# Picurit/cutter-vad

Hardware: AMD Instinct MI355X
Metric: 512-sample frames/sec, Silero V5 16kHz, batch=8192 streams per GPU (higher is better)
Workload: dtype f32

## Files before the change

### cutter_vad_amd/csrc/engine.cpp

```cpp
#include "../../include/vad_engine.h"

#include <hip/hip_runtime_api.h>

#include <algorithm>
#include <atomic>
#include <cmath>
#include <condition_variable>
#include <cstdarg>
#include <cstdlib>
#include <new>
#include <chrono>
#include <cstring>
#include <deque>
#include <mutex>
#include <string>
#include <thread>
#include <unordered_map>
#include <array>
#include <vector>

#include "pack_weights.h"
#include "resample_generic.h"
#include "vad_layout.h"

extern "C" hipError_t vadk_launch_silero_v5(const vadk::StepParams *p, hipStream_t stream);
extern "C" hipError_t vadk_launch_silero_v4(const vadk::StepParams *p, hipStream_t stream);
extern "C" hipError_t vadk_launch_silero_v5_t16(const vadk::StepParams *p, hipStream_t stream);
extern "C" hipError_t vadk_launch_silero_v4_t16(const vadk::StepParams *p, int one_per_cu, hipStream_t stream);
extern "C" hipError_t vadk_launch_silero_v5_t16_rates(const vadk::StepParams *p, const vadk::RateParams *r, hipStream_t stream);
extern "C" hipError_t vadk_launch_silero_v5_scan16(const vadk::StepParams *p, const vadk::ScanItem *items, const vadk::ScanArgs *a,
                                                   hipStream_t stream);
extern "C" hipError_t vadk_launch_scan_cut(const vadk::CutArgs *a, hipStream_t stream);
extern "C" hipError_t vadk_launch_scan_segments(const vadk::SegArgs *a, hipStream_t stream);
extern "C" hipError_t vadk_launch_scan_resample(const vadk::ScanResampleArgs *a, hipStream_t stream);
extern "C" hipError_t vadk_launch_resample(const vadk::ResampleParams *p, hipStream_t stream);
extern "C" hipError_t vadk_launch_slot_control(vadk::SmSlot *sm, float *state, const int32_t *d_slots, int n, int op,
                                               const vadk::SmSlot *def, const vad_thresholds *d_thr, int nthr, hipStream_t stream);
extern "C" hipError_t vadk_launch_sm_replay(vadk::SmSlot *sm, int slot, const float *probs, int n, uint8_t *events,
                                            int32_t *seg, hipStream_t stream);
extern "C" hipError_t vadk_launch_g711_expand(const void *d_in, int16_t *d_out, int64_t nbytes, int alaw, hipStream_t stream);

namespace {
// ... 98 lines not shown
    int16_t *d_g711 = nullptr; size_t d_g711_cap = 0;
    static constexpr size_t SMALL_BYTES = 256u << 10;
    uint8_t *h_small_in = nullptr, *h_small_out = nullptr;
    std::vector<void *> host_blocks;
    uint8_t *d_small_in = nullptr, *d_small_out = nullptr;
    vadk::StepParams base{};
    static constexpr int T16_MAX_STREAMS = 4096;
    float *d_wstream16 = nullptr;
    size_t wbytes16 = 0;
    float *d_wstream16x = nullptr;
    size_t wbytes16x = 0;
    float *d_wstream16y = nullptr;
    size_t wbytes16y = 0;
    uint32_t sect16[vadk::NWAVES][16] = {};
    int tile_policy = 0;
    bool rates_fused = true;
    bool shared_gpu = false;
    int sample_rate = 16000;
    int frame_samples = VAD_FRAME_SAMPLES;
    std::vector<int32_t> work_index;
    std::vector<uint8_t> work_kind;
    std::vector<int64_t> work_samples;
    uint8_t *h_ctl = nullptr, *d_ctl = nullptr; size_t ctl_cap = 0;
    static constexpr int PIPE_DEPTH = 2;
    struct PipeBuf {
        void *d_frames = nullptr; size_t d_frames_cap = 0;
        uint8_t *d_io = nullptr, *h_io = nullptr; size_t io_cap = 0;
        hipEvent_t copied = nullptr, done = nullptr, out = nullptr;
        int64_t ticket = -1; int64_t n = 0; int32_t T = 0; bool busy = false, collecting = false;
    } pipe[PIPE_DEPTH];
// ... 373 lines not shown
        p16.wstream_x_bytes = (uint32_t)e->wbytes16x;
        p16.wstream_y = e->d_wstream16y;
        p16.wstream_y_bytes = (uint32_t)e->wbytes16y;
        std::memcpy(p16.sect, e->sect16, sizeof p16.sect);
        const int tiles16 = (p.n + 15) / 16;
        r = vadk_launch_silero_v4_t16(&p16, (!e->shared_gpu && tiles16 <= e->prop.multiProcessorCount) ? 1 : 0, s);
    } else if (e->version == 5 && t16) {
        vadk::StepParams p16 = p;
        p16.wstream = e->d_wstream16;
        p16.wstream_bytes = (uint32_t)e->wbytes16;
        p16.wstream_x = e->d_wstream16x;
        p16.wstream_x_bytes = (uint32_t)e->wbytes16x;
        p16.wstream_y = e->d_wstream16y;
        p16.wstream_y_bytes = (uint32_t)e->wbytes16y;
        std::memcpy(p16.sect, e->sect16, sizeof p16.sect);
        r = vadk_launch_silero_v5_t16(&p16, s);
    } else if (e->version == 5) r = vadk_launch_silero_v5(&p, s);
    else if (e->version == 4) r = vadk_launch_silero_v4(&p, s);
    if (r != hipSuccess) return e->hip_fail(r, "kernel launch");
    e->steps += 1;
    e->frames += (int64_t)p.n * p.T;
    return VAD_OK;
}

int step_host(vad_engine *e, const int64_t *slots, int64_t n, int32_t T, const void *frames, int fmt, float thr,
              float *probs, uint8_t *events, int32_t *seg) {
    if (!e) return VAD_ERR_INVALID_ARG;
    std::lock_guard<std::mutex> lk(e->mu);
    if (n < 0 || T < 1 || (n > 0 && (!slots || !frames || !probs)))
        return e->fail(VAD_ERR_INVALID_ARG, "Model prediction failed: null buffer or bad count");
// ... 2611 lines not shown
            g_create_error = "vad_debug_pack_weights: output buffer too small";
            return VAD_ERR_INVALID_ARG;
        }
        std::memcpy(out, pw.data.data(), pw.data.size() * sizeof(float));
    }
    return VAD_OK;
}

int vad_debug_set_tile(vad_engine *e, int32_t streams_per_tile) {
    if (!e) return VAD_ERR_INVALID_ARG;
    std::lock_guard<std::mutex> lk(e->mu);
    if (streams_per_tile == -1 || streams_per_tile == -2) {
        e->rates_fused = streams_per_tile == -2;
        return VAD_OK;
    }
    if (streams_per_tile != 0 && streams_per_tile != 16 && streams_per_tile != 32)
        return e->fail(VAD_ERR_INVALID_ARG, "tile: 0 (by batch size), 16 or 32");
    if (streams_per_tile == 16 && !e->d_wstream16)
        return e->fail(VAD_ERR_UNSUPPORTED, "Silero V5's 8 kHz sub-model has no 16-stream tile kernel");
    e->tile_policy = streams_per_tile;
    return VAD_OK;
}

int vad_debug_sm_replay(vad_engine *e, int64_t slot, const float *probs, int64_t n, uint8_t *events_out,
                        int32_t *seg_frames_out) {
    if (!e || !probs || !events_out || !seg_frames_out || n < 1) return VAD_ERR_INVALID_ARG;
    std::lock_guard<std::mutex> lk(e->mu);
    if (slot < 0 || slot >= e->max_streams || !e->open[(size_t)slot])
        return e->fail(VAD_ERR_BAD_SLOT, "slot %lld is not an open stream", (long long)slot);
    HIP_TRY(e, hipSetDevice(e->device));
    if (int rc = ensure(e, e->d_probs, e->d_probs_cap, sizeof(float) * n)) return rc;
    if (int rc = ensure(e, e->d_events, e->d_events_cap, (size_t)n)) return rc;
    if (int rc = ensure(e, e->d_seg, e->d_seg_cap, sizeof(int32_t) * n)) return rc;
    HIP_TRY(e, hipMemcpyAsync(e->d_probs, probs, sizeof(float) * n, hipMemcpyHostToDevice, e->stream));
    HIP_TRY(e, hipStreamSynchronize(e->stream));
// ... 40 lines not shown
```

### cutter_vad_amd/csrc/silero_v5_t16.hip

```cpp
#include <hip/hip_runtime.h>
#include <type_traits>
#include <utility>
#include "vad_layout.h"
#include "sm_device.h"
#include "vadk_device.h"

using namespace vadk;

#ifdef VADK_STAMPS
#define STAMP(k)                                                                                   \
    do {                                                                                           \
        if (lane == 0) P.stamps[((size_t)blockIdx.x * NWAVES + w) * 32 + (k)] = clock64();          \
    } while (0)
template <class V>
__device__ __forceinline__ void stamp_wait(V v) {
    if constexpr (sizeof(V) == 4) asm volatile("" ::"v"(v) : "memory");
    else if constexpr (sizeof(V) == 32) asm volatile("" ::"v"(v.b.x) : "memory");
    else asm volatile("" ::"v"(v.x) : "memory");
}
#define STAMP_ON(k, v)                                                                             \
    do {                                                                                           \
        if constexpr (!RS) {                                                                       \
            stamp_wait(v);                                                                         \
            STAMP(k);                                                                              \
        }                                                                                          \
    } while (0)
#define STAMP_DRAIN(k)                                                                             \
// ... 82 lines not shown
        if constexpr (k_ == 7) { F_[0] = N_[0]; F_[1] = N_[1]; F_[2] = N_[2]; }                                 \
        if constexpr (!(FOLD(u)) || k_ == 7) SB();                                                              \
    }
#define X3_STEP(s, B, SRC, EXTRA, FOLD)                                                                         \
    X3_UNIT(8 * (s) + 0, B, SRC, EXTRA, FOLD) X3_UNIT(8 * (s) + 1, B, SRC, EXTRA, FOLD)                         \
    X3_UNIT(8 * (s) + 2, B, SRC, EXTRA, FOLD) X3_UNIT(8 * (s) + 3, B, SRC, EXTRA, FOLD)                         \
    X3_UNIT(8 * (s) + 4, B, SRC, EXTRA, FOLD) X3_UNIT(8 * (s) + 5, B, SRC, EXTRA, FOLD)                         \
    X3_UNIT(8 * (s) + 6, B, SRC, EXTRA, FOLD) X3_UNIT(8 * (s) + 7, B, SRC, EXTRA, FOLD)
#define X3_HALF(B, SRC, EXTRA, FOLD)                                                                            \
    {                                                                                                           \
        u32x4 F_[3], N_[3];                                                                                     \
        _Pragma("unroll") for (int p_ = 0; p_ < 3; ++p_) F_[p_] = PL_RD(SRC, 0, p_);                            \
        SB();                                                                                                   \
        X3_STEP(0, B, SRC, EXTRA, FOLD) X3_STEP(1, B, SRC, EXTRA, FOLD)                                         \
        X3_STEP(2, B, SRC, EXTRA, FOLD) X3_STEP(3, B, SRC, EXTRA, FOLD)                                         \
    }
#define X3_CONV(NS, NT, STR, NO, LDM, B, U0, SRC, ACC, EXTRA)                                         \
    {                                                                                                           \
        constexpr int NU_ = (NS) * 3 * (NT);                                                                    \
        u32x4 F_[3][3], N_[3][3];                                                                               \
        _Pragma("unroll") for (int c_ = 0; c_ < 3; ++c_)                                                        \
            _Pragma("unroll") for (int p_ = 0; p_ < 3; ++p_) F_[c_][p_] = PL_RD(SRC(c_), 0, p_);                \
        SB();                                                                                                   \
        x3_units([&](auto uc_) {                                                                                \
            constexpr int u_ = decltype(uc_)::value, s_ = u_ / (3 * (NT)), r_ = u_ % (3 * (NT));                \
            constexpr int t_ = r_ / (NT), tl_ = r_ % (NT);                                                      \
            if constexpr (u_ + X3_D < NU_) { LDM((B) + 3 * (u_ + X3_D), (U0) + u_ + X3_D) }                     \
            if constexpr (r_ == 0 && s_ + 1 < (NS)) {                                                           \
                _Pragma("unroll") for (int c_ = 0; c_ < 3; ++c_)                                                \
                    _Pragma("unroll") for (int p_ = 0; p_ < 3; ++p_) N_[c_][p_] = PL_RD(SRC(c_), s_ + 1, p_);   \
// ... 8 lines not shown
                    _Pragma("unroll") for (int c_ = 0; c_ < 3; ++c_)                                            \
                        _Pragma("unroll") for (int p_ = 0; p_ < 3; ++p_) F_[c_][p_] = N_[c_][p_];               \
                }                                                                                               \
            }                                                                                                   \
            SB();                                                                                               \
        }, std::make_integer_sequence<int, NU_>{});                                                             \
    }

#define STEP16_PARAMS const float *k_wstream, float *k_state, SmSlot *k_sm, const int32_t *k_slots, const void *k_frames, const int k_n, \
                      const uint32_t k_wstream_bytes, const int k_T, const StepParams P, const RateParams R
#define STEP16_NO_SCAN                                  \
    constexpr bool SCAN = false;                        \
    constexpr int CH = 1;                               \
    constexpr const ScanItem *k_items = nullptr;        \
    constexpr ScanArgs S{};
template <bool F32IN_, bool RS, bool K8 = false, bool ONE = false>
__global__ void __launch_bounds__(NTHREADS, 1) silero_v5_step16(STEP16_PARAMS) {
    constexpr int FMT = F32IN_ ? 0 : 1;
    STEP16_NO_SCAN
#include "silero_v5_t16_body.h"
}
template <bool ALAW, bool K8, bool ONE>
__global__ void __launch_bounds__(NTHREADS, 1) silero_v5_step16_g711(STEP16_PARAMS) {
    constexpr int FMT = ALAW ? 3 : 2;
    constexpr bool RS = false;
    STEP16_NO_SCAN
#include "silero_v5_t16_body.h"
}
template <int FMT_, bool K8>
__global__ void __launch_bounds__(NTHREADS, 1) silero_v5_scan16(const float *k_wstream, float *k_state, SmSlot *k_sm, const ScanItem *k_items,
                                                                const void *k_frames, const int k_n, const uint32_t k_wstream_bytes,
                                                                const int k_T, const StepParams P, const ScanArgs S) {
    constexpr int FMT = FMT_;
    constexpr bool RS = false, ONE = false, SCAN = true;
    constexpr int CH = 1;
    constexpr const int32_t *k_slots = nullptr;
    const RateParams R{};
#include "silero_v5_t16_body.h"
}
template <int FMT_, bool K8>
__global__ void __launch_bounds__(NTHREADS, 1) silero_v5_stereo16(const float *k_wstream, float *k_state, SmSlot *k_sm, const ScanItem *k_items,
                                                                  const void *k_frames, const int k_n, const uint32_t k_wstream_bytes,
                                                                  const int k_T, const StepParams P, const ScanArgs S) {
    constexpr int FMT = FMT_;
    constexpr bool RS = false, ONE = false, SCAN = true;
    constexpr int CH = 2;
    constexpr const int32_t *k_slots = nullptr;
    const RateParams R{};
#include "silero_v5_t16_body.h"
}
#undef STEP16_NO_SCAN
#undef STEP16_PARAMS
#undef X3_CONV
#undef X3_HALF
#undef X3_STEP
#undef X3_UNIT
#undef PL_RD


#define V5_ARGS p->wstream, p->state, p->sm, p->slots, p->frames, (int)p->n, p->wstream_bytes, (int)p->T, *p
extern "C" hipError_t vadk_launch_silero_v5_t16(const vadk::StepParams *p, hipStream_t stream) {
    (void)hipGetLastError();
    const int tiles = (p->n + MT16 - 1) / MT16;
    if (tiles <= 0) return hipSuccess;
    const vadk::RateParams none{};
#define T16_LAUNCH(F, K, O) hipLaunchKernelGGL((silero_v5_step16<F, false, K, O>), dim3(tiles), dim3(vadk::NTHREADS), 0, stream, V5_ARGS, none)
    if (p->T < 1) return hipErrorInvalidValue;
    const bool k8 = p->variant != 0;
// ... 10 lines not shown
            else { if (one) T16_LAUNCH_G711(false, false, true); else T16_LAUNCH_G711(false, false, false); }
        }
        return hipGetLastError();
    }
    if (p->fmt < 0 || p->fmt > 2) return hipErrorInvalidValue;
    const bool f32 = p->fmt == 0;
    if (k8) {
        if (f32) { if (one) T16_LAUNCH(true, true, true); else T16_LAUNCH(true, true, false); }
        else { if (one) T16_LAUNCH(false, true, true); else T16_LAUNCH(false, true, false); }
    } else {
        if (f32) { if (one) T16_LAUNCH(true, false, true); else T16_LAUNCH(true, false, false); }
        else { if (one) T16_LAUNCH(false, false, true); else T16_LAUNCH(false, false, false); }
    }
#undef T16_LAUNCH_G711
#undef T16_LAUNCH
    return hipGetLastError();
}

extern "C" hipError_t vadk_launch_silero_v5_scan16(const vadk::StepParams *p, const vadk::ScanItem *items, const vadk::ScanArgs *a,
                                                   hipStream_t stream) {
    (void)hipGetLastError();
    const int tiles = (p->n + MT16 - 1) / MT16;
    if (tiles <= 0) return hipSuccess;
    if (p->T < 1 || p->fmt < 0 || p->fmt > 4 || a->hopq < 1 || a->t0 < 0 || (a->audio_bytes >> 31)) return hipErrorInvalidValue;
    if ((reinterpret_cast<uintptr_t>(p->frames) & 3) || (reinterpret_cast<uintptr_t>(items) & 15)) return hipErrorInvalidValue;
    if (a->channels < 0 || a->channels > 2 || (a->channels == 2 && (reinterpret_cast<uintptr_t>(p->frames) & 7))) return hipErrorInvalidValue;
#define SCAN16_LAUNCH(F, K)                                                                                                    \
    hipLaunchKernelGGL((silero_v5_scan16<F, K>), dim3(tiles), dim3(vadk::NTHREADS), 0, stream, p->wstream, p->state, p->sm, items, \
                       p->frames, (int)p->n, p->wstream_bytes, (int)p->T, *p, *a)
#define STEREO16_LAUNCH(F, K)                                                                                                  \
// ... 27 lines not shown
```

### cutter_vad_amd/csrc/silero_v5_t16_body.h

```cpp
#define KP(f) k_##f
    using namespace vadk::v5;
    constexpr bool F32IN = FMT == 0;
    constexpr bool G711 = FMT >= 2;
    static_assert(!RS || F32IN, "resampled frames are float32");
    static_assert(!(RS && K8), "the fused resampler feeds the 16 kHz model");
    static_assert(!SCAN || (!RS && !ONE), "a scan is the frame-loop form on audio in HBM");
    static_assert(CH == 1 || (CH == 2 && SCAN), "two interleaved channels: whole recordings only");
    constexpr int QL = K8 ? 8 : 16;
    constexpr int CS = 4 * QL;
    constexpr int PP = K8 ? 24 : 48;
    __shared__ f32x4 lds[T_LDS_F4 + (RS ? MT16 * FQ : 0) + (F32IN ? T_FLAG_F4 : 0)];
    f32x4 *const RX = lds;
    f32x4 *const RE = lds + T_ROW_E * QSD;
    f32x4 *const RP0 = lds + T_ROW_E0 * QSD;
    f32x4 *const RH = lds + T_ROW_H * QSD;
    float *const headp = reinterpret_cast<float *>(RH + T_ROWS_H * QSD);
    float *const nyqv = headp + 64;
    float *const fcor = nyqv + 48;
    constexpr int FCOR_SINK = 144;
    SmSlot *const smL = reinterpret_cast<SmSlot *>(fcor + 144 + 64);
    f32x4 *const biasL = reinterpret_cast<f32x4 *>(smL + MT16);
    uint8_t *const flagL = reinterpret_cast<uint8_t *>(lds + T_LDS_F4 + (RS ? MT16 * FQ : 0));

    const int tid = threadIdx.x;
    const int lane = tid & 63;
    const int w = __builtin_amdgcn_readfirstlane(tid >> 6);
    if constexpr (!RS) STAMP(19);
    const int n = lane & 15;
    const int kq = lane >> 4;
    const int nq = kq * QSD + n;
    const int nqL = kq * QSL + n;
    const int vcol = (int)blockIdx.x * MT16 + n;
    int gf = vcol;
    bool live = vcol < KP(n);
    if constexpr (RS) {
        int s0 = R.seg[0].stream0, vs = 0;
#pragma unroll
        for (int k = 1; k < RATE_MAX_SEGS; ++k)
            if (k < R.nseg && vcol >= R.seg[k].vstart) { s0 = R.seg[k].stream0; vs = R.seg[k].vstart; }
        gf = s0 + vcol - vs;
        live = vcol < R.total;
    }
    const int tile0 = (int)blockIdx.x * MT16;
    int slot, ncol = 0;
    uint32_t obase = 0;
    if constexpr (SCAN) {
        const u32x4 it = live ? *reinterpret_cast<const u32x4 *>(k_items + vcol) : u32x4{0u, 0u, 0u, 0u};
        slot = (int)it.x;
        ncol = (int)it.z - S.t0;
        obase = it.w + (uint32_t)S.t0;
    } else {
        slot = live ? (KP(slots) ? KP(slots)[gf] : gf) : 0;
    }
    const __amdgpu_buffer_rsrc_t wrs = __builtin_amdgcn_make_buffer_rsrc(const_cast<float *>(KP(wstream)), 0, (int)KP(wstream_bytes), 0x00020000);
    const int lane16 = lane * 16;
#define WL(blk) ldw(wrs, lane16, (blk))
    const __amdgpu_buffer_rsrc_t wrx = __builtin_amdgcn_make_buffer_rsrc(const_cast<float *>(P.wstream_x), 0, (int)P.wstream_x_bytes, 0x00020000);
#define WX(blk) ldw(wrx, lane16, (blk))
// ... 21 lines not shown
        SCAN ? (int)S.audio_bytes : (int)((unsigned)KP(n) * (unsigned)T * ((f32in ? 2048u : G711 ? 512u : 1024u) >> (K8 ? 1 : 0))), 0x00020000);
    constexpr int X_NT = K8 ? 0 : 2;
    struct XQ2F { u32x4 a, b; };
    using XQ = std::conditional_t<CH == 2, std::conditional_t<f32in, XQ2F, std::conditional_t<G711, u32x2, u32x4>>,
                                  std::conditional_t<G711, uint32_t, u32x4>>;
    auto x_load = [&](int off) -> XQ {
        if constexpr (CH == 2 && f32in)
            return XQ2F{__builtin_amdgcn_raw_buffer_load_b128(frs, off, 0, X_NT), __builtin_amdgcn_raw_buffer_load_b128(frs, off + 16, 0, X_NT)};
        else if constexpr (CH == 2 && G711) return __builtin_amdgcn_raw_buffer_load_b64(frs, off, 0, X_NT);
        else if constexpr (G711) return __builtin_amdgcn_raw_buffer_load_b32(frs, off, 0, X_NT);
        else return __builtin_amdgcn_raw_buffer_load_b128(frs, off, 0, X_NT);
    };
    XQ xa_[4], xb_[4], xc_[4];
    constexpr bool XCARRY = !RS && !K8;
#define X_K0(c) ((XCARRY && (c) > 0) ? 2 : 0)
    f32x4 *const F4 = lds + T_LDS_F4;
    uint32_t xq0 = 0;
    [[maybe_unused]] uint32_t xmode = 0;
    if constexpr (SCAN) {
        const int li = tile0 + lms;
        if constexpr (CH == 2) {
            const uint32_t qm = li < KP(n) ? k_items[li].quad0 : 0u;
            xmode = qm >> SCAN_MODE_SHIFT;
            xq0 = (qm & ((1u << SCAN_MODE_SHIFT) - 1u)) + (uint32_t)S.t0 * S.hopq;
        } else {
        xq0 = (li < KP(n) ? k_items[li].quad0 : 0u) + (uint32_t)S.t0 * S.hopq;
        }
    }
#define X_ISSUE(c, XR, tt)                                                                                      \
    if constexpr (RS) {                                                                                         \
        _Pragma("unroll") for (int k = 0; k < 4; ++k)                                                           \
// ... 83 lines not shown
#pragma unroll
    for (int rt = 0; rt < 2; ++rt) hv[rt] = *reinterpret_cast<const f32x4 *>(KP(state) + (size_t)slot * 256 + 32 * w + 16 * rt + 4 * kq);
    SB();
    auto bias2 = __builtin_amdgcn_raw_buffer_load_b64(wrs, lane * 8, (o_l + T_LSTM_BIAS_BLOCK) * 1024, 0);
    const bool sm_thread = (tid < MT16) && live;
    const int sm_slot = slot;
    f32x4 smq[6];
    if (tid < MT16) {
#pragma unroll
        for (int k = 0; k < 6; ++k) smq[k] = reinterpret_cast<const f32x4 *>(KP(sm) + slot)[k];
    }
    SB();
    f32x4 xw[X3_NR][3];
#define X3_LDR(blk, slot) _Pragma("unroll") for (int p_ = 0; p_ < 3; ++p_) xw[(slot) % X3_NR][p_] = WL((blk) + p_);
#define X3_LD(B, u) X3_LDR((B) + 3 * (u), (u))
#define X3_LDX(blk, slot) _Pragma("unroll") for (int p_ = 0; p_ < 3; ++p_) xw[(slot) % X3_NR][p_] = WX((blk) + p_);
#define X3_LDY(blk, slot) _Pragma("unroll") for (int p_ = 0; p_ < 3; ++p_) xw[(slot) % X3_NR][p_] = WY((blk) + p_);
#define H_FIRSTX(tt)                                                                                            \
    {                                                                                                           \
        if constexpr (K8) { X_ISSUE8(0, xa_, tt) X_ISSUE8(2, xb_, tt) }                                         \
        else { X_ISSUE(0, xa_, tt) X_ISSUE(1, xb_, tt) }                                                        \
    }
#define H_FIRST(L, tt, WITHX)                                                                                   \
    {                                                                                                           \
        _Pragma("unroll") for (int u_ = 0; u_ < X3_D; ++u_) { X3_LD((L) + LSTM_X3_HALF_BLOCKS, u_) }             \
        if constexpr (WITHX) H_FIRSTX(tt)                                                                       \
        SB();                                                                                                   \
        if constexpr (RS) { X_ISSUE(2, xc_, tt) SB(); }                                                         \
    }
    if constexpr (!RS) STAMP(29);
    if constexpr (!RS) H_FIRST(o_x3, 0, K8)
    const f32x4 W1 = ldw(wrs, q * 16, o_nyq), W3 = ldw(wrs, (2 * QL + q) * 16, o_nyq);
    const float w64 = ldw(wrs, QL * 16, o_nyq).x;
    f32x4 cst[2];
#pragma unroll
    for (int rt = 0; rt < 2; ++rt) cst[rt] = *reinterpret_cast<const f32x4 *>(KP(state) + (size_t)slot * 256 + 128 + 32 * w + 16 * rt + 4 * kq);
    bool chunk0_requested = false;
    if constexpr (RS) {
        if (cur.valid && cur.S.wstream != nullptr && cur.S.n_in == 1536) {
            if (cur.shape == 0) load_chunk(std::integral_constant<int, 0>{}, cur, 0, xlA);
// ... 297 lines not shown
          else if (cur.shape == 1) run_part(std::integral_constant<int, 1>{});
          else if (cur.shape == 2) run_part(std::integral_constant<int, 2>{});
          else run_part(std::integral_constant<int, 3>{});
#undef OL
        }
        __syncthreads();
        cur = mk_part(cur.sk + 1);
        }
    }

    STAMP(0);
    for (int t = 0;;) {
        int ws_stft = o_stft, ws_x0 = o_x0, ws_y1 = o_y1, ws_e2 = o_e2, ws_e3 = o_e3, ws_l = o_l, ws_x3 = o_x3;
        asm volatile("" : "+s"(ws_stft), "+s"(ws_x0), "+s"(ws_y1), "+s"(ws_e2), "+s"(ws_e3), "+s"(ws_l), "+s"(ws_x3));
        f32x4 G[8];
        {
            const int wh = ws_x3 + LSTM_X3_HALF_BLOCKS;
            f32x4 xcA, xcB;
            float xm = 0.f;
            auto decode = [&](XQ b) -> f32x4 {
                f32x4 v;
                if constexpr (CH == 2) {
                    f32x4 dl, dr;
                    if constexpr (G711) {
                        dl = g711_quad<FMT == 3>(__builtin_amdgcn_perm(b.y, b.x, 0x06040200u));
                        dr = g711_quad<FMT == 3>(__builtin_amdgcn_perm(b.y, b.x, 0x07050301u));
                    } else if constexpr (!f32in) {
                        dl = f32x4{i16_div((int)(short)(b.x & 0xffffu), sc, rsc), i16_div((int)(short)(b.y & 0xffffu), sc, rsc),
                                   i16_div((int)(short)(b.z & 0xffffu), sc, rsc), i16_div((int)(short)(b.w & 0xffffu), sc, rsc)};
                        dr = f32x4{i16_div((int)(short)(b.x >> 16), sc, rsc), i16_div((int)(short)(b.y >> 16), sc, rsc),
// ... 77 lines not shown
        const int er = (q < 8 ? 64 * (c) + 32 + q : T_FOLD_SINK - 8 + q) * QSL + ms;                            \
        st2(&RX[er], pep);                                                                                      \
        st2(&RX[er + 8 * QSL], pen);                                                                            \
        st2(&RX[er + 16 * QSL], qen);                                                                           \
        st2(&RX[er + 24 * QSL], qep);                                                                           \
        }                                                                                                       \
    }
#define H_MIX                                                                                                   \
    _Pragma("unroll") for (int i_ = 0; i_ < 6; ++i_) {                                                          \
        __builtin_amdgcn_sched_group_barrier(0x008, 3, 0);                                                      \
        __builtin_amdgcn_sched_group_barrier(0x002, 28, 0);                                                     \
    }
            if constexpr (RS) H_FIRST(ws_x3, t, true)
            {
                const f32x4 *const bq = biasL + 32 * w + kq;
#pragma unroll
                for (int k = 0; k < 8; ++k) G[k] = bq[(k >> 1) * 8 + (k & 1) * 4];
            }
            __syncthreads();
            STAMP(31);
#define H_EXTRA(u)                                                                                              \
            if constexpr ((u) == 2 && !RS && !K8) { X_ISSUE(2, xc_, t) }                                        \
            if constexpr ((u) == 15) { if constexpr (K8) { X_FOLD(lcol, xa_, 0) } else { X_FOLD(0, xa_, 0) } H_MIX }   \
            if constexpr ((u) == 23) { if constexpr (K8) { X_FOLD(2, xb_, 1) X_FLAG } else { X_FOLD(1, xb_, 1) } H_MIX }   \
            if constexpr ((u) == 31 && !K8) { X_FOLD(2, xc_, 2) X_FLAG H_MIX }
#define H_FOLDREGION(u) (((u) & 7) >= 5 && (u) >= 8 && ((u) < 24 || !K8))
            X3_HALF(wh, RH, H_EXTRA, H_FOLDREGION)
#undef H_EXTRA
#undef H_FOLDREGION
#undef H_MIX
#undef X_FOLD
#undef X_FLAG
        }
        f32x4 Sw[2];
#pragma unroll
        for (int k = 0; k < 2; ++k) Sw[k] = WL(ws_stft + k);
        SB();
        STAMP(1);
        __syncthreads();
        STAMP(2);

        {
// ... 1 lines not shown
            const int c = pair >> 4, ms = pair & 15;
            float a = 0.f;
            if (pair < 48) {
#pragma unroll
                for (int i = 0; i < 2; ++i) {
                    const f32x4 pp = RX[(CS * c + (K8 ? 0 : 32) + pt * 2 + i) * QSL + ms];
                    a += (pp.x - pp.y) + (pp.z - pp.w);
                }
            }
            a += __shfl_xor(a, 1);
            a += __shfl_xor(a, 2);
            if (pair < 48 && pt == 0) nyqv[c * 16 + ms] = fabsf(a + fcor[(c * 3 + 0) * 16 + ms] + fcor[(c * 3 + 1) * 16 + ms]);
        }

        f32x4 e0f[ENC0_X3_F32_BLOCKS];
#define E0_FIRST                                                                                                \
    _Pragma("unroll") for (int k = 0; k < ENC0_X3_F32_BLOCKS; ++k) e0f[k] = WX(ws_x0 + k);                      \
    _Pragma("unroll") for (int u_ = 0; u_ < X3_D; ++u_) { X3_LDX(ws_x0 + ENC0_X3_F32_BLOCKS + 3 * u_, u_) }
        if constexpr (K8) {
            const bool even = w < 2;
            f32x4 sre[3], sim[3];
#pragma unroll
            for (int c = 0; c < 3; ++c) {
                const float y128 = fcor[(c * 3 + 0) * 16 + n], a64 = fcor[(c * 3 + 1) * 16 + n], b64 = fcor[(c * 3 + 2) * 16 + n];
                const float rp = even ? y128 + a64 : -y128, rm = even ? y128 - a64 : -y128;
                const float ip = even ? 0.f : -b64, im_ = even ? 0.f : b64;
                sre[c] = f32x4{rp, rm, rp, rm};
                sim[c] = f32x4{ip, im_, ip, im_};
            }
            const int rR = even ? 0 : QL, rI = even ? 2 * QL : 3 * QL;
            const f32x4 wr0 = Sw[0], wi0 = Sw[1], wr1 = WL(ws_stft + 2), wi1 = WL(ws_stft + 3);
#pragma unroll
            for (int j = 0; j < 2; ++j) {
// ... 67 lines not shown
#undef S_MMA
#undef S_ROW_R
#undef S_ROW_I
            E0_FIRST
            SB();
            __syncthreads();
#pragma unroll
            for (int c = 0; c < 3; ++c)
                st_planes(RX + (PP * c + 12 * w) * QSD + nq, pk::mag(are[c][0], aim[c][0]), pk::mag(are[c][1], aim[c][1]));
        }
#undef E0_FIRST
        STAMP(3);
        __syncthreads();
        STAMP(4);

        constexpr int NU0 = (K8 ? 2 : 4) * 3 * 2;
        f32x4 e1b;
        {
            f32x4 acc[3][2];
            {
                const float nv[3] = {nyqv[n], nyqv[16 + n], nyqv[32 + n]};
#pragma unroll
                for (int o = 0; o < 3; ++o)
#pragma unroll
                    for (int rt = 0; rt < 2; ++rt) {
                        f32x4 a = e0f[rt];
#pragma unroll
                        for (int t = 0; t < 3; ++t)
                            if (o + t - 1 >= 0 && o + t - 1 < 3) a = pk::fma(e0f[2 + 2 * t + rt], pk::splat(nv[o + t - 1]), a);
                        acc[o][rt] = a;
                    }
            }
#define E0_SRC(c) (RX + PP * (c) * QSD)
#define E0_EXTRA(u)                                                                                             \
            if constexpr ((u) == NU0 - X3_D) e1b = WY(ws_y1);                                                   \
            if constexpr ((u) + X3_D >= NU0) { X3_LDY(ws_y1 + ENC1_X3_F32_BLOCKS + 3 * ((u) + X3_D - NU0), (u) + X3_D) }
            X3_CONV(K8 ? 2 : 4, 2, 1, 3, X3_LDX, ws_x0 + ENC0_X3_F32_BLOCKS, 0, E0_SRC, acc, E0_EXTRA)
#undef E0_SRC
#undef E0_EXTRA
#pragma unroll
            for (int c = 0; c < 3; ++c) st_planes(RP0 + (48 * c + 12 * w) * QSD + nq, relu4(acc[c][0]), relu4(acc[c][1]));
        }
        STAMP(5);
        __syncthreads();
        STAMP(6);

        f32x4 e2b[2], E2w[2], e3b[2], E3w[2];
        {
            constexpr int NU1 = 4 * 3;
            f32x4 acc[2][1] = {{e1b}, {e1b}};
#define E1_SRC(c) (RP0 + 48 * (c) * QSD)
#define E1_EXTRA(u)                                                                                             \
            if constexpr ((u) == NU1 - X3_D) {         \
                const int ge = 2 + 8 * (w >> 1);                                                                \
                e2b[0] = WL(ws_e2); e2b[1] = WL(ws_e2 + 1);                                                     \
                E2w[0] = WL(ws_e2 + ge); E2w[1] = WL(ws_e2 + ge + 1);                                           \
                e3b[0] = WL(ws_e3); e3b[1] = WL(ws_e3 + 1);                                                     \
// ... 32 lines not shown
        STAMP(10);

        {
            const int ws = ws_e3 + 2;
            f32x4 acc[2] = {e3b[0], e3b[1]};
            f32x4 wv[8], av[4];
            wv[0] = E3w[0]; wv[1] = E3w[1];
#pragma unroll
            for (int k = 2; k < 8; ++k) wv[k] = WL(ws + k);
#pragma unroll
            for (int j = 0; j < 4; ++j) {
                const f32x4 a = RE[(4 * j) * QSD + nq], b2 = RE[(16 + 4 * j) * QSD + nq];
                av[j] = relu4(f32x4{a.x + b2.x, a.y + b2.y, a.z + b2.z, a.w + b2.w});
            }
#pragma unroll
            for (int u = 0; u < X3_D; ++u) { X3_LD(ws_x3, u) }
            SB();
#pragma unroll
            for (int j = 0; j < 4; ++j) { acc[0] = mfma16(wv[2 * j], av[j], acc[0]); acc[1] = mfma16(wv[2 * j + 1], av[j], acc[1]); }
            st_planes(RX + 12 * w * QSD + nq, relu4(acc[0]), relu4(acc[1]));
        }
        STAMP(11);
        __syncthreads();
        STAMP(12);

        {
            const int ws = ws_l + 8;
            f32x4 hw[2];
#define L_EXTRA(u) if constexpr ((u) == 24) { hw[0] = WL(ws + 128); hw[1] = WL(ws + 129); }
#define L_FOLDREGION(u) false
            X3_HALF(ws_x3, RX, L_EXTRA, L_FOLDREGION)
#undef L_EXTRA
#undef L_FOLDREGION
            STAMP(18);
            STAMP(13);
            __syncthreads();
            STAMP(14);
            f32x4 part4 = f32x4{0.f, 0.f, 0.f, 0.f};
            const bool rej = f32in && (K8 ? (flagL[n] | flagL[16 + n]) : flagL[n]) != 0;
            const bool bad = SCAN ? (rej || t >= ncol) : rej;
            f32x4 hq[2];
#pragma unroll
            for (int rt = 0; rt < 2; ++rt) {
                const f32x4 i4 = G[0 + rt], f4 = G[2 + rt], g4 = G[4 + rt], o4 = G[6 + rt], c4 = cst[rt], hwv = hw[rt];
                f32x4 cn = pk::fma(pk::sigmoid4(f4), c4, pk::mul(pk::sigmoid4(i4), pk::tanh4(g4)));
                f32x4 hn = pk::mul(pk::sigmoid4(o4), pk::tanh4(cn));
                part4 = pk::fma(hwv, relu4(hn), part4);
                if constexpr ((f32in || SCAN) && !ONE && !RS) {
                    hn = bad ? hv[rt] : hn;
                    cn = bad ? c4 : cn;
                    hv[rt] = hn;
                }
// ... 35 lines not shown
                SmSlot sm = smL[tid];
                int seg = 0;
                const int ev = bad ? EV_REJECTED : sm_step(sm, p, &seg);
                if (t == T - 1) { if (!((ONE || RS) && bad)) KP(sm)[sm_slot] = sm; }
                else smL[tid] = sm;
                if (ev & 2) seg_last = seg;
                if (P.events) P.events[(size_t)gf * T + t] = (uint8_t)ev;
                }
            }
        }
        if (++t >= T) break;
        if constexpr (!RS) H_FIRST(ws_x3, t, true)
    }
#undef H_FIRST
#undef H_FIRSTX
#undef X3_LD
#undef X3_LDR
#undef X3_LDX
#undef X3_LDY
#undef WY
#undef WX
#undef X_ISSUE
#undef X_K0
#undef WL
    if constexpr (!SCAN) { if (sm_thread && P.seg_frames) P.seg_frames[gf] = seg_last; }
    if constexpr (!RS) STAMP(27);
    STAMP_DRAIN(28);
#undef KP
```

Baseline: 218.9 million.

## Add paired-tile Silero V5 kernel that splits weight loads across two tiles per block

Adds a 512-thread kernel variant in which each block processes two 16-stream tiles. Each half loads only half of the LSTM and encoder-0 weight blocks and computes its output columns for both tiles, reading the other tile's activations from shared LDS and exchanging gate partials through LDS. The aim is to halve per-wave weight streaming, which dominates the one-frame step, at the cost of doubled LDS per block and extra cross-half exchanges. It is enabled by default for single-frame f32/int16 calls when the tile count exceeds the CU count.

```diff
diff --git a/cutter_vad_amd/csrc/engine.cpp b/cutter_vad_amd/csrc/engine.cpp
--- a/cutter_vad_amd/csrc/engine.cpp
+++ b/cutter_vad_amd/csrc/engine.cpp
@@ -26,6 +26,7 @@
 extern "C" hipError_t vadk_launch_silero_v5(const vadk::StepParams *p, hipStream_t stream);
 extern "C" hipError_t vadk_launch_silero_v4(const vadk::StepParams *p, hipStream_t stream);
 extern "C" hipError_t vadk_launch_silero_v5_t16(const vadk::StepParams *p, hipStream_t stream);
+extern "C" hipError_t vadk_launch_silero_v5_t16_pair(const vadk::StepParams *p, hipStream_t stream);
 extern "C" hipError_t vadk_launch_silero_v4_t16(const vadk::StepParams *p, int one_per_cu, hipStream_t stream);
 extern "C" hipError_t vadk_launch_silero_v5_t16_rates(const vadk::StepParams *p, const vadk::RateParams *r, hipStream_t stream);
 extern "C" hipError_t vadk_launch_silero_v5_scan16(const vadk::StepParams *p, const vadk::ScanItem *items, const vadk::ScanArgs *a,
@@ -154,6 +155,7 @@
     size_t wbytes16y = 0;
     uint32_t sect16[vadk::NWAVES][16] = {};
     int tile_policy = 0;
+    int pair_policy = 0;
     bool rates_fused = true;
     bool shared_gpu = false;
     int sample_rate = 16000;
@@ -557,6 +559,11 @@
         p16.wstream_y = e->d_wstream16y;
         p16.wstream_y_bytes = (uint32_t)e->wbytes16y;
         std::memcpy(p16.sect, e->sect16, sizeof p16.sect);
+        const int tiles16 = (int)((p.n + 15) / 16);
+        const bool pairable = p.T == 1 && p.variant == 0 && p.fmt >= 0 && p.fmt <= 2;
+        if (pairable && (e->pair_policy > 0 || (e->pair_policy == 0 && tiles16 > e->prop.multiProcessorCount)))
+            r = vadk_launch_silero_v5_t16_pair(&p16, s);
+        else
         r = vadk_launch_silero_v5_t16(&p16, s);
     } else if (e->version == 5) r = vadk_launch_silero_v5(&p, s);
     else if (e->version == 4) r = vadk_launch_silero_v4(&p, s);
@@ -3198,11 +3205,16 @@
         e->rates_fused = streams_per_tile == -2;
         return VAD_OK;
     }
+    if (streams_per_tile == -3 || streams_per_tile == -4) {
+        e->pair_policy = streams_per_tile == -3 ? 1 : -1;
+        return VAD_OK;
+    }
     if (streams_per_tile != 0 && streams_per_tile != 16 && streams_per_tile != 32)
         return e->fail(VAD_ERR_INVALID_ARG, "tile: 0 (by batch size), 16 or 32");
     if (streams_per_tile == 16 && !e->d_wstream16)
         return e->fail(VAD_ERR_UNSUPPORTED, "Silero V5's 8 kHz sub-model has no 16-stream tile kernel");
     e->tile_policy = streams_per_tile;
+    e->pair_policy = 0;
     return VAD_OK;
 }
 
diff --git a/cutter_vad_amd/csrc/silero_v5_t16.hip b/cutter_vad_amd/csrc/silero_v5_t16.hip
--- a/cutter_vad_amd/csrc/silero_v5_t16.hip
+++ b/cutter_vad_amd/csrc/silero_v5_t16.hip
@@ -10,7 +10,7 @@
 #ifdef VADK_STAMPS
 #define STAMP(k)                                                                                   \
     do {                                                                                           \
-        if (lane == 0) P.stamps[((size_t)blockIdx.x * NWAVES + w) * 32 + (k)] = clock64();          \
+        if (lane == 0) P.stamps[((size_t)tilei * NWAVES + w) * 32 + (k)] = clock64();          \
     } while (0)
 template <class V>
 __device__ __forceinline__ void stamp_wait(V v) {
@@ -123,6 +123,30 @@
         SB();                                                                                                   \
         X3_STEP(0, B, SRC, EXTRA, FOLD) X3_STEP(1, B, SRC, EXTRA, FOLD)                                         \
         X3_STEP(2, B, SRC, EXTRA, FOLD) X3_STEP(3, B, SRC, EXTRA, FOLD)                                         \
+    }
+#define X3P_UNIT(v, B, SRC0, SRC1, EXTRA, FOLD)                                                                 \
+    {                                                                                                           \
+        constexpr int s_ = (v) >> 2, q_ = (v) & 3;                                                              \
+        if constexpr ((v) + X3_D < 16) { X3_LDP(B, (v) + X3_D) }                                                \
+        if constexpr (q_ == 0 && s_ < 3) {                                                                      \
+            _Pragma("unroll") for (int p_ = 0; p_ < 3; ++p_) { N0_[p_] = PL_RD(SRC0, s_ + 1, p_); N1_[p_] = PL_RD(SRC1, s_ + 1, p_); } \
+        }                                                                                                       \
+        EXTRA(v)                                                                                                \
+        Gp[q_][0] = mfma_x3(xw[(v) % X3_NR], F0_, Gp[q_][0]);                                                   \
+        Gp[q_][1] = mfma_x3(xw[(v) % X3_NR], F1_, Gp[q_][1]);                                                   \
+        if constexpr (q_ == 3) { _Pragma("unroll") for (int p_ = 0; p_ < 3; ++p_) { F0_[p_] = N0_[p_]; F1_[p_] = N1_[p_]; } } \
+        if constexpr (!(FOLD(v)) || q_ == 3) SB();                                                              \
+    }
+#define X3P_STEP(s, B, SRC0, SRC1, EXTRA, FOLD)                                                                 \
+    X3P_UNIT(4 * (s) + 0, B, SRC0, SRC1, EXTRA, FOLD) X3P_UNIT(4 * (s) + 1, B, SRC0, SRC1, EXTRA, FOLD)         \
+    X3P_UNIT(4 * (s) + 2, B, SRC0, SRC1, EXTRA, FOLD) X3P_UNIT(4 * (s) + 3, B, SRC0, SRC1, EXTRA, FOLD)
+#define X3P_HALF(B, SRC0, SRC1, EXTRA, FOLD)                                                                    \
+    {                                                                                                           \
+        u32x4 F0_[3], F1_[3], N0_[3], N1_[3];                                                                   \
+        _Pragma("unroll") for (int p_ = 0; p_ < 3; ++p_) { F0_[p_] = PL_RD(SRC0, 0, p_); F1_[p_] = PL_RD(SRC1, 0, p_); } \
+        SB();                                                                                                   \
+        X3P_STEP(0, B, SRC0, SRC1, EXTRA, FOLD) X3P_STEP(1, B, SRC0, SRC1, EXTRA, FOLD)                         \
+        X3P_STEP(2, B, SRC0, SRC1, EXTRA, FOLD) X3P_STEP(3, B, SRC0, SRC1, EXTRA, FOLD)                         \
     }
 #define X3_CONV(NS, NT, STR, NO, LDM, B, U0, SRC, ACC, EXTRA)                                         \
     {                                                                                                           \
@@ -161,9 +185,18 @@
     constexpr int CH = 1;                               \
     constexpr const ScanItem *k_items = nullptr;        \
     constexpr ScanArgs S{};
+#define STEP16_NO_PAIR constexpr bool PAIR = false;
 template <bool F32IN_, bool RS, bool K8 = false, bool ONE = false>
 __global__ void __launch_bounds__(NTHREADS, 1) silero_v5_step16(STEP16_PARAMS) {
     constexpr int FMT = F32IN_ ? 0 : 1;
+    STEP16_NO_SCAN
+    STEP16_NO_PAIR
+#include "silero_v5_t16_body.h"
+}
+template <bool F32IN_>
+__global__ void __launch_bounds__(2 * NTHREADS, 1) silero_v5_pair16(STEP16_PARAMS) {
+    constexpr int FMT = F32IN_ ? 0 : 1;
+    constexpr bool RS = false, K8 = false, ONE = true, PAIR = true;
     STEP16_NO_SCAN
 #include "silero_v5_t16_body.h"
 }
@@ -172,6 +205,7 @@
     constexpr int FMT = ALAW ? 3 : 2;
     constexpr bool RS = false;
     STEP16_NO_SCAN
+    STEP16_NO_PAIR
 #include "silero_v5_t16_body.h"
 }
 template <int FMT_, bool K8>
@@ -183,6 +217,7 @@
     constexpr int CH = 1;
     constexpr const int32_t *k_slots = nullptr;
     const RateParams R{};
+    STEP16_NO_PAIR
 #include "silero_v5_t16_body.h"
 }
 template <int FMT_, bool K8>
@@ -194,11 +229,16 @@
     constexpr int CH = 2;
     constexpr const int32_t *k_slots = nullptr;
     const RateParams R{};
-#include "silero_v5_t16_body.h"
-}
+    STEP16_NO_PAIR
+#include "silero_v5_t16_body.h"
+}
+#undef STEP16_NO_PAIR
 #undef STEP16_NO_SCAN
 #undef STEP16_PARAMS
 #undef X3_CONV
+#undef X3P_HALF
+#undef X3P_STEP
+#undef X3P_UNIT
 #undef X3_HALF
 #undef X3_STEP
 #undef X3_UNIT
@@ -239,6 +279,17 @@
     }
 #undef T16_LAUNCH_G711
 #undef T16_LAUNCH
+    return hipGetLastError();
+}
+
+extern "C" hipError_t vadk_launch_silero_v5_t16_pair(const vadk::StepParams *p, hipStream_t stream) {
+    (void)hipGetLastError();
+    const int tiles = (p->n + MT16 - 1) / MT16;
+    if (tiles <= 0) return hipSuccess;
+    if (p->T != 1 || p->variant != 0 || p->fmt < 0 || p->fmt > 2) return hipErrorInvalidValue;
+    const vadk::RateParams none{};
+    if (p->fmt == 0) hipLaunchKernelGGL((silero_v5_pair16<true>), dim3((tiles + 1) / 2), dim3(2 * vadk::NTHREADS), 0, stream, V5_ARGS, none);
+    else hipLaunchKernelGGL((silero_v5_pair16<false>), dim3((tiles + 1) / 2), dim3(2 * vadk::NTHREADS), 0, stream, V5_ARGS, none);
     return hipGetLastError();
 }
 
diff --git a/cutter_vad_amd/csrc/silero_v5_t16_body.h b/cutter_vad_amd/csrc/silero_v5_t16_body.h
--- a/cutter_vad_amd/csrc/silero_v5_t16_body.h
+++ b/cutter_vad_amd/csrc/silero_v5_t16_body.h
@@ -6,31 +6,38 @@
     static_assert(!(RS && K8), "the fused resampler feeds the 16 kHz model");
     static_assert(!SCAN || (!RS && !ONE), "a scan is the frame-loop form on audio in HBM");
     static_assert(CH == 1 || (CH == 2 && SCAN), "two interleaved channels: whole recordings only");
+    static_assert(!PAIR || (ONE && !RS && !K8 && !G711 && !SCAN), "paired tiles: one-frame calls of the 16 kHz model, float32 / int16");
     constexpr int QL = K8 ? 8 : 16;
     constexpr int CS = 4 * QL;
     constexpr int PP = K8 ? 24 : 48;
-    __shared__ f32x4 lds[T_LDS_F4 + (RS ? MT16 * FQ : 0) + (F32IN ? T_FLAG_F4 : 0)];
-    f32x4 *const RX = lds;
-    f32x4 *const RE = lds + T_ROW_E * QSD;
-    f32x4 *const RP0 = lds + T_ROW_E0 * QSD;
-    f32x4 *const RH = lds + T_ROW_H * QSD;
+    constexpr int LDS_HALF = T_LDS_F4 + (RS ? MT16 * FQ : 0) + (F32IN ? T_FLAG_F4 : 0);
+    static_assert(!PAIR || 2 * LDS_HALF * 16 <= 160 * 1024, "both halves' LDS on one CU");
+    __shared__ f32x4 lds[(PAIR ? 2 : 1) * LDS_HALF];
+    const int hf = PAIR ? __builtin_amdgcn_readfirstlane((int)threadIdx.x >> 8) : 0;
+    f32x4 *const ldsH = PAIR ? lds + hf * LDS_HALF : lds;
+    [[maybe_unused]] f32x4 *const ldsO = PAIR ? lds + (1 - hf) * LDS_HALF : lds;
+    f32x4 *const RX = ldsH;
+    f32x4 *const RE = ldsH + T_ROW_E * QSD;
+    f32x4 *const RP0 = ldsH + T_ROW_E0 * QSD;
+    f32x4 *const RH = ldsH + T_ROW_H * QSD;
     float *const headp = reinterpret_cast<float *>(RH + T_ROWS_H * QSD);
     float *const nyqv = headp + 64;
     float *const fcor = nyqv + 48;
     constexpr int FCOR_SINK = 144;
     SmSlot *const smL = reinterpret_cast<SmSlot *>(fcor + 144 + 64);
     f32x4 *const biasL = reinterpret_cast<f32x4 *>(smL + MT16);
-    uint8_t *const flagL = reinterpret_cast<uint8_t *>(lds + T_LDS_F4 + (RS ? MT16 * FQ : 0));
-
-    const int tid = threadIdx.x;
+    uint8_t *const flagL = reinterpret_cast<uint8_t *>(ldsH + T_LDS_F4 + (RS ? MT16 * FQ : 0));
+
+    const int tid = PAIR ? (int)threadIdx.x & 255 : (int)threadIdx.x;
     const int lane = tid & 63;
     const int w = __builtin_amdgcn_readfirstlane(tid >> 6);
+    [[maybe_unused]] const int tilei = PAIR ? 2 * (int)blockIdx.x + hf : (int)blockIdx.x;
     if constexpr (!RS) STAMP(19);
     const int n = lane & 15;
     const int kq = lane >> 4;
     const int nq = kq * QSD + n;
     const int nqL = kq * QSL + n;
-    const int vcol = (int)blockIdx.x * MT16 + n;
+    const int vcol = (PAIR ? tilei : (int)blockIdx.x) * MT16 + n;
     int gf = vcol;
     bool live = vcol < KP(n);
     if constexpr (RS) {
@@ -41,7 +48,7 @@
         gf = s0 + vcol - vs;
         live = vcol < R.total;
     }
-    const int tile0 = (int)blockIdx.x * MT16;
+    const int tile0 = (PAIR ? tilei : (int)blockIdx.x) * MT16;
     int slot, ncol = 0;
     uint32_t obase = 0;
     if constexpr (SCAN) {
@@ -93,7 +100,7 @@
     XQ xa_[4], xb_[4], xc_[4];
     constexpr bool XCARRY = !RS && !K8;
 #define X_K0(c) ((XCARRY && (c) > 0) ? 2 : 0)
-    f32x4 *const F4 = lds + T_LDS_F4;
+    f32x4 *const F4 = ldsH + T_LDS_F4;
     uint32_t xq0 = 0;
     [[maybe_unused]] uint32_t xmode = 0;
     if constexpr (SCAN) {
@@ -207,6 +214,8 @@
     f32x4 xw[X3_NR][3];
 #define X3_LDR(blk, slot) _Pragma("unroll") for (int p_ = 0; p_ < 3; ++p_) xw[(slot) % X3_NR][p_] = WL((blk) + p_);
 #define X3_LD(B, u) X3_LDR((B) + 3 * (u), (u))
+#define X3_LDP(B, v) X3_LDR((B) + 3 * (8 * ((v) >> 2) + 2 * ((v) & 3) + hf), (v))
+#define X3_LDU(B, u) if constexpr (PAIR) { X3_LDP(B, u) } else { X3_LD(B, u) }
 #define X3_LDX(blk, slot) _Pragma("unroll") for (int p_ = 0; p_ < 3; ++p_) xw[(slot) % X3_NR][p_] = WX((blk) + p_);
 #define X3_LDY(blk, slot) _Pragma("unroll") for (int p_ = 0; p_ < 3; ++p_) xw[(slot) % X3_NR][p_] = WY((blk) + p_);
 #define H_FIRSTX(tt)                                                                                            \
@@ -216,7 +225,7 @@
     }
 #define H_FIRST(L, tt, WITHX)                                                                                   \
     {                                                                                                           \
-        _Pragma("unroll") for (int u_ = 0; u_ < X3_D; ++u_) { X3_LD((L) + LSTM_X3_HALF_BLOCKS, u_) }             \
+        _Pragma("unroll") for (int u_ = 0; u_ < X3_D; ++u_) { X3_LDU((L) + LSTM_X3_HALF_BLOCKS, u_) }            \
         if constexpr (WITHX) H_FIRSTX(tt)                                                                       \
         SB();                                                                                                   \
         if constexpr (RS) { X_ISSUE(2, xc_, tt) SB(); }                                                         \
@@ -544,6 +553,7 @@
         int ws_stft = o_stft, ws_x0 = o_x0, ws_y1 = o_y1, ws_e2 = o_e2, ws_e3 = o_e3, ws_l = o_l, ws_x3 = o_x3;
         asm volatile("" : "+s"(ws_stft), "+s"(ws_x0), "+s"(ws_y1), "+s"(ws_e2), "+s"(ws_e3), "+s"(ws_l), "+s"(ws_x3));
         f32x4 G[8];
+        [[maybe_unused]] f32x4 Gp[4][2];
         {
             const int wh = ws_x3 + LSTM_X3_HALF_BLOCKS;
             f32x4 xcA, xcB;
@@ -651,8 +661,13 @@
             if constexpr (RS) H_FIRST(ws_x3, t, true)
             {
                 const f32x4 *const bq = biasL + 32 * w + kq;
+                if constexpr (PAIR) {
+#pragma unroll
+                    for (int k = 0; k < 4; ++k) Gp[k][0] = Gp[k][1] = bq[k * 8 + hf * 4];
+                } else {
 #pragma unroll
                 for (int k = 0; k < 8; ++k) G[k] = bq[(k >> 1) * 8 + (k & 1) * 4];
+                }
             }
             __syncthreads();
             STAMP(31);
@@ -662,7 +677,25 @@
             if constexpr ((u) == 23) { if constexpr (K8) { X_FOLD(2, xb_, 1) X_FLAG } else { X_FOLD(1, xb_, 1) } H_MIX }   \
             if constexpr ((u) == 31 && !K8) { X_FOLD(2, xc_, 2) X_FLAG H_MIX }
 #define H_FOLDREGION(u) (((u) & 7) >= 5 && (u) >= 8 && ((u) < 24 || !K8))
+#define HP_MIX                                                                                                  \
+    _Pragma("unroll") for (int i_ = 0; i_ < 6; ++i_) {                                                          \
+        __builtin_amdgcn_sched_group_barrier(0x008, 4, 0);                                                      \
+        __builtin_amdgcn_sched_group_barrier(0x002, 28, 0);                                                     \
+    }
+#define HP_EXTRA(v)                                                                                             \
+            if constexpr ((v) == 1) { X_ISSUE(2, xc_, t) }                                                      \
+            if constexpr ((v) == 7) { X_FOLD(0, xa_, 0) HP_MIX }                                                \
+            if constexpr ((v) == 11) { X_FOLD(1, xb_, 1) HP_MIX }                                               \
+            if constexpr ((v) == 15) { X_FOLD(2, xc_, 2) X_FLAG HP_MIX }
+#define HP_FOLDREGION(v) (((v) & 3) >= 2 && (v) >= 4)
+            if constexpr (PAIR) {
+                X3P_HALF(wh, RH, (ldsO + T_ROW_H * QSD), HP_EXTRA, HP_FOLDREGION)
+            } else {
             X3_HALF(wh, RH, H_EXTRA, H_FOLDREGION)
+            }
+#undef HP_EXTRA
+#undef HP_FOLDREGION
+#undef HP_MIX
 #undef H_EXTRA
 #undef H_FOLDREGION
 #undef H_MIX
@@ -694,9 +727,16 @@
         }
 
         f32x4 e0f[ENC0_X3_F32_BLOCKS];
+#define E0P_BLK(v) (ws_x0 + ENC0_X3_F32_BLOCKS + 3 * (2 * (v) + hf))
 #define E0_FIRST                                                                                                \
+    if constexpr (PAIR) {                                                                                       \
+        e0f[0] = WX(ws_x0 + hf);                                                                                \
+        _Pragma("unroll") for (int k = 0; k < 3; ++k) e0f[1 + k] = WX(ws_x0 + 2 + 2 * k + hf);                  \
+        _Pragma("unroll") for (int u_ = 0; u_ < X3_D; ++u_) { X3_LDX(E0P_BLK(u_), u_) }                         \
+    } else {                                                                                                    \
     _Pragma("unroll") for (int k = 0; k < ENC0_X3_F32_BLOCKS; ++k) e0f[k] = WX(ws_x0 + k);                      \
-    _Pragma("unroll") for (int u_ = 0; u_ < X3_D; ++u_) { X3_LDX(ws_x0 + ENC0_X3_F32_BLOCKS + 3 * u_, u_) }
+    _Pragma("unroll") for (int u_ = 0; u_ < X3_D; ++u_) { X3_LDX(ws_x0 + ENC0_X3_F32_BLOCKS + 3 * u_, u_) }     \
+    }
         if constexpr (K8) {
             const bool even = w < 2;
             f32x4 sre[3], sim[3];
@@ -794,9 +834,72 @@
         __syncthreads();
         STAMP(4);
 
-        constexpr int NU0 = (K8 ? 2 : 4) * 3 * 2;
+        constexpr int NU0 = (K8 ? 2 : 4) * 3 * (PAIR ? 1 : 2);
         f32x4 e1b;
-        {
+#define E0_EXTRA(u)                                                                                             \
+            if constexpr ((u) == NU0 - X3_D) e1b = WY(ws_y1);                                                   \
+            if constexpr ((u) + X3_D >= NU0) { X3_LDY(ws_y1 + ENC1_X3_F32_BLOCKS + 3 * ((u) + X3_D - NU0), (u) + X3_D) }
+        if constexpr (PAIR) {
+            f32x4 acc[3][2];
+            const float *const nyqO = reinterpret_cast<const float *>(ldsO + (T_ROW_H + T_ROWS_H) * QSD) + 64;
+#pragma unroll
+            for (int st = 0; st < 2; ++st) {
+                const float *const nq_ = st ? nyqO : nyqv;
+                const float nv[3] = {nq_[n], nq_[16 + n], nq_[32 + n]};
+#pragma unroll
+                for (int o = 0; o < 3; ++o) {
+                    f32x4 a = e0f[0];
+#pragma unroll
+                    for (int t = 0; t < 3; ++t)
+                        if (o + t - 1 >= 0 && o + t - 1 < 3) a = pk::fma(e0f[1 + t], pk::splat(nv[o + t - 1]), a);
+                    acc[o][st] = a;
+                }
+            }
+#define E0P_SRC(st, c) (((st) ? ldsO : RX) + PP * (c) * QSD)
+            u32x4 F_[2][3][3], N1_[2][3];
+#pragma unroll
+            for (int st = 0; st < 2; ++st)
+#pragma unroll
+                for (int c_ = 0; c_ < 3; ++c_)
+#pragma unroll
+                    for (int p_ = 0; p_ < 3; ++p_) F_[st][c_][p_] = PL_RD(E0P_SRC(st, c_), 0, p_);
+            SB();
+            x3_units([&](auto uc_) {
+                constexpr int v_ = decltype(uc_)::value, s_ = v_ / 3, t_ = v_ % 3;
+                if constexpr (v_ + X3_D < NU0) { X3_LDX(E0P_BLK(v_ + X3_D), v_ + X3_D) }
+                if constexpr (t_ == 1 && s_ + 1 < 4) {
+#pragma unroll
+                    for (int st = 0; st < 2; ++st)
+#pragma unroll
+                        for (int p_ = 0; p_ < 3; ++p_) N1_[st][p_] = PL_RD(E0P_SRC(st, 1), s_ + 1, p_);
+                }
+                E0_EXTRA(v_)
+#pragma unroll
+                for (int o_ = 0; o_ < 3; ++o_) {
+                    const int c_ = o_ + t_ - 1;
+                    if (c_ >= 0 && c_ < 3) {
+#pragma unroll
+                        for (int st = 0; st < 2; ++st) acc[o_][st] = mfma_x3(xw[v_ % X3_NR], F_[st][c_], acc[o_][st]);
+                    }
+                }
+                if constexpr (s_ + 1 < 4 && t_ >= 1) {
+#pragma unroll
+                    for (int st = 0; st < 2; ++st)
+#pragma unroll
+                        for (int p_ = 0; p_ < 3; ++p_) {
+                            if constexpr (t_ == 1) F_[st][0][p_] = PL_RD(E0P_SRC(st, 0), s_ + 1, p_);
+                            else { F_[st][1][p_] = N1_[st][p_]; F_[st][2][p_] = PL_RD(E0P_SRC(st, 2), s_ + 1, p_); }
+                        }
+                }
+                SB();
+            }, std::make_integer_sequence<int, NU0>{});
+#undef E0P_SRC
+#pragma unroll
+            for (int st = 0; st < 2; ++st)
+#pragma unroll
+                for (int c = 0; c < 3; ++c)
+                    st_planes_half((st ? ldsO : ldsH) + (T_ROW_E0 + 48 * c + 12 * w) * QSD + nq, hf, relu4(acc[c][st]));
+        } else {
             f32x4 acc[3][2];
             {
                 const float nv[3] = {nyqv[n], nyqv[16 + n], nyqv[32 + n]};
@@ -812,15 +915,13 @@
                     }
             }
 #define E0_SRC(c) (RX + PP * (c) * QSD)
-#define E0_EXTRA(u)                                                                                             \
-            if constexpr ((u) == NU0 - X3_D) e1b = WY(ws_y1);                                                   \
-            if constexpr ((u) + X3_D >= NU0) { X3_LDY(ws_y1 + ENC1_X3_F32_BLOCKS + 3 * ((u) + X3_D - NU0), (u) + X3_D) }
             X3_CONV(K8 ? 2 : 4, 2, 1, 3, X3_LDX, ws_x0 + ENC0_X3_F32_BLOCKS, 0, E0_SRC, acc, E0_EXTRA)
 #undef E0_SRC
+#pragma unroll
+            for (int c = 0; c < 3; ++c) st_planes(RP0 + (48 * c + 12 * w) * QSD + nq, relu4(acc[c][0]), relu4(acc[c][1]));
+        }
 #undef E0_EXTRA
-#pragma unroll
-            for (int c = 0; c < 3; ++c) st_planes(RP0 + (48 * c + 12 * w) * QSD + nq, relu4(acc[c][0]), relu4(acc[c][1]));
-        }
+#undef E0P_BLK
         STAMP(5);
         __syncthreads();
         STAMP(6);
@@ -883,7 +984,7 @@
                 av[j] = relu4(f32x4{a.x + b2.x, a.y + b2.y, a.z + b2.z, a.w + b2.w});
             }
 #pragma unroll
-            for (int u = 0; u < X3_D; ++u) { X3_LD(ws_x3, u) }
+            for (int u = 0; u < X3_D; ++u) { X3_LDU(ws_x3, u) }
             SB();
 #pragma unroll
             for (int j = 0; j < 4; ++j) { acc[0] = mfma16(wv[2 * j], av[j], acc[0]); acc[1] = mfma16(wv[2 * j + 1], av[j], acc[1]); }
@@ -898,13 +999,31 @@
             f32x4 hw[2];
 #define L_EXTRA(u) if constexpr ((u) == 24) { hw[0] = WL(ws + 128); hw[1] = WL(ws + 129); }
 #define L_FOLDREGION(u) false
+#define LP_EXTRA(v) if constexpr ((v) == 12) { hw[0] = WL(ws + 128); hw[1] = WL(ws + 129); }
+            if constexpr (PAIR) {
+                X3P_HALF(ws_x3, RX, ldsO, LP_EXTRA, L_FOLDREGION)
+                f32x4 *const hb = ldsO + (T_ROW_E0 + 16 * w) * QSD + nq;
+#pragma unroll
+                for (int k = 0; k < 4; ++k) hb[4 * k * QSD] = Gp[k][1];
+            } else {
             X3_HALF(ws_x3, RX, L_EXTRA, L_FOLDREGION)
+            }
+#undef LP_EXTRA
 #undef L_EXTRA
 #undef L_FOLDREGION
             STAMP(18);
             STAMP(13);
             __syncthreads();
             STAMP(14);
+            if constexpr (PAIR) {
+                const f32x4 *const hb = ldsH + (T_ROW_E0 + 16 * w) * QSD + nq;
+#pragma unroll
+                for (int k = 0; k < 4; ++k) {
+                    const f32x4 o = hb[4 * k * QSD];
+                    G[2 * k] = hf ? o : Gp[k][0];
+                    G[2 * k + 1] = hf ? Gp[k][0] : o;
+                }
+            }
             f32x4 part4 = f32x4{0.f, 0.f, 0.f, 0.f};
             const bool rej = f32in && (K8 ? (flagL[n] | flagL[16 + n]) : flagL[n]) != 0;
             const bool bad = SCAN ? (rej || t >= ncol) : rej;
@@ -970,6 +1089,8 @@
     }
 #undef H_FIRST
 #undef H_FIRSTX
+#undef X3_LDU
+#undef X3_LDP
 #undef X3_LD
 #undef X3_LDR
 #undef X3_LDX
```

After: 228.3 million, median of 6. 1.04x the previous value.
